# peter-seres/python-ray-tracer

Measured on AMD Instinct MI355X. Metric: Mrays/sec + frame time (ms) at 1920x1080, 8 spheres, depth=3, higher is better.
Workload: dtype f64

## Files before the change

python-ray-tracer_amd/csrc/mi355rt.hip:

```cpp
#include "../../include/mi355rt.h"
#include "rt_device.h"
#include "rt_bloom.h"
#include "rt_denoise.h"
#include "rt_denoise_var.h"
#include "rt_feedback.h"
#include "rt_film.h"
#include "rt_film_launch.h"
#include "rt_geometry.h"
#include "rt_guides.h"
#include "rt_launch.h"
#include "rt_plan.h"
#include "rt_scene.h"
#include "rt_streams.h"
#include "rt_temporal.h"

#include <cmath>
#include <cstdio>
#include <cstdlib>
#include <algorithm>
#include <array>
#include <cstring>
#include <memory>
#include <new>
#include <string>
// ... 40 lines not shown
        }
    };
    std::unique_ptr<Pipeline> pipe;
    int chunk_mode = -1;
    int cluster_min = rt::CLUSTER_MIN;
    int lanes_primary = 1;
    rt::PlanKnobs knobs;
    int render_chunks = 4;
    int log_kernels = 0;
    int remeasure = 24;
    struct Slot {
        hipStream_t stream = nullptr;
        Buf u8, f32;
    } slots[RT_RENDER_SLOTS];
    hipEvent_t ev0 = nullptr, ev1 = nullptr;
    Buf scene[RT_SCENE_RING];
    int scene_cur = 0;
    Buf pixel_loc, u8, f32;
    rt::SceneLayout lay;
    Buf texels[RT_SCENE_RING];
    bool have_scene = false;
    rt::View view;
    size_t lds_limit_set[rt::FAMILIES] = {};
    size_t guides_lds_set = 0;
    unsigned *tile_stats = nullptr;
    struct Feedback : rt::FeedbackSlot {
        Buf cost, gtmp, btmp, order[2];
    } fbs[RT_FEEDBACK_SLOTS];
    rt::FeedbackBook book;
    rt_ctx() { for (int i = 0; i < RT_FEEDBACK_SLOTS; ++i) book.slot[i] = &fbs[i]; }
    template <class F> void own_streams(F f)
    {
        if (stream) f(stream);
        for (Slot &sl : slots) if (sl.stream) f(sl.stream);
        if (pipe) pipe->streams(f);
    }
    ~rt_ctx()
    {
        for (auto &f : fbs)
            for (void *e : rt::release_events(f)) (void)hipEventDestroy((hipEvent_t)e);
        pipe.reset();
        own_streams([](hipStream_t s) { (void)hipStreamDestroy(s); });
        for (hipEvent_t e : {ev0, ev1}) if (e) (void)hipEventDestroy(e);
    }
    rt_stats stats = {};
    Buf counts;
// ... 37 lines not shown
int check_params(rt_ctx *ctx, const rt_params *p, int x0, int x1) { return refuse(ctx, rt::check_params(ctx->have_scene, ctx->view, ctx->lay, p, x0, x1)); }

hipStream_t stream_of(rt_ctx *ctx, void *stream) { return stream ? (hipStream_t)stream : ctx->stream; }

using StreamRecord = rt::StreamBook<Buf>::Record;

int stream_record(rt_ctx *ctx, hipStream_t stream, StreamRecord **out)
{
    const int rc = ctx->streams.record(stream, out);
    if (rc != RT_OK) return fail(ctx, rc, ctx->streams.NO_MEMORY);
    ctx->streams.reads_scene(**out, ctx->scene_cur);
    return RT_OK;
}

int raise_lds(rt_ctx *ctx, const void *const *fns, size_t n, size_t lds, size_t &set)
{
    if (lds <= 48 * 1024 || lds <= set) return RT_OK;
    for (size_t i = 0; i < n; ++i)
        if (fns[i]) RT_HIP(ctx, hipFuncSetAttribute(fns[i], hipFuncAttributeMaxDynamicSharedMemorySize, (int)lds));
    set = lds;
    return RT_OK;
}

using rt::Shape; using rt::SHAPES; using rt::NSHAPES; using rt::has_kernel;

template <rt::Family F, int I>
const void *kernel_at()
{
    constexpr Shape s = SHAPES[I];
    if constexpr (has_kernel(F, s))
        return (const void *)rt::render_kernel<s.aa, s.park, s.wpw, s.count, s.lat, s.mode, F>;
    else
        return nullptr;
}
template <rt::Family F, int... I>
std::array<const void *, NSHAPES> family_kernels(std::integer_sequence<int, I...>)
{
    return {kernel_at<F, I>()...};
}

constexpr std::make_integer_sequence<int, NSHAPES> ALL_SHAPES{};
const std::array<const void *, NSHAPES> KERNELS[rt::FAMILIES] = {
    family_kernels<rt::Family::PLAIN>(ALL_SHAPES), family_kernels<rt::Family::MAT>(ALL_SHAPES),
    family_kernels<rt::Family::REFR>(ALL_SHAPES),  family_kernels<rt::Family::SCAT>(ALL_SHAPES),
    family_kernels<rt::Family::SOFT>(ALL_SHAPES),  family_kernels<rt::Family::LENS>(ALL_SHAPES),
    family_kernels<rt::Family::LENS_SOFT>(ALL_SHAPES),
    family_kernels<rt::Family::TEX_SCAT>(ALL_SHAPES), family_kernels<rt::Family::TEX_SOFT>(ALL_SHAPES),
    family_kernels<rt::Family::TEX_LENS>(ALL_SHAPES), family_kernels<rt::Family::TEX_LENS_SOFT>(ALL_SHAPES),
    family_kernels<rt::Family::LIT_SCAT>(ALL_SHAPES), family_kernels<rt::Family::LIT_SOFT>(ALL_SHAPES),
    family_kernels<rt::Family::LIT_LENS>(ALL_SHAPES), family_kernels<rt::Family::LIT_LENS_SOFT>(ALL_SHAPES),
    family_kernels<rt::Family::SKY_SCAT>(ALL_SHAPES), family_kernels<rt::Family::SKY_SOFT>(ALL_SHAPES),
    family_kernels<rt::Family::SKY_LENS>(ALL_SHAPES), family_kernels<rt::Family::SKY_LENS_SOFT>(ALL_SHAPES),
};
static_assert(rt::FAMILIES == 19 && (int)rt::Family::TEX_LENS_SOFT == 10 && (int)rt::Family::LIT_LENS_SOFT == 14 &&
              (int)rt::Family::SKY_SCAT == 15 && (int)rt::Family::SKY_LENS_SOFT == 18,
              "KERNELS lists the families in enum order");

int stream_buffer(rt_ctx *ctx, Buf &b, hipStream_t stream, size_t bytes, bool sync)
{
    if (sync) RT_HIP(ctx, hipStreamSynchronize(stream));
    return ensure(ctx, b, bytes);
}

int acquire_tables(rt_ctx *ctx, StreamRecord &sr, const rt::KParams &k, const float **out)
{
    const hipStream_t stream = (hipStream_t)sr.stream;
    const rt::TableKey key = rt::table_key(ctx->scene_epoch, k.anchors, k.floor_anch, k.cam_o);
    const size_t bytes = rt::table_floats(k.S, k.NC, k.anchors, false, true, k.P) * sizeof(float);
    const rt::TableDecision d = ctx->streams.tables(sr, key, bytes);
    Buf &b = sr.buf[rt::BUF_TABLES0 + d.set];
    if (d.rebuild) {
        int rc = stream_buffer(ctx, b, stream, d.bytes, d.sync);
        if (rc != RT_OK) return rc;
        hipLaunchKernelGGL(rt::tables_kernel, dim3(1), dim3(rt::TABLE_THREADS), 0, stream, k, (float *)b.p);
        ctx->stats.table_builds++;
        RT_HIP(ctx, hipGetLastError());
// ... 111 lines not shown

int switch_order(rt_ctx *ctx, Feedback &f)
{
    if (!f.building) return RT_OK;
    const hipError_t q = hipEventQuery((hipEvent_t)f.done);
    if (q != hipSuccess) {
        (void)hipGetLastError();
        return RT_OK;
    }
    for (void *us : rt::switch_order(f)) {
        hipEvent_t ev = (hipEvent_t)rt::take_spare(f);
        if (!ev) RT_HIP(ctx, hipEventCreateWithFlags(&ev, hipEventDisableTiming));
        RT_HIP(ctx, hipEventRecord(ev, (hipStream_t)us));
        rt::add_fence(f, us, ev);
    }
    return RT_OK;
}

int launch_one(rt_ctx *ctx, rt::KParams &k, const rt::LaunchPlan &plan, const rt_geo_plan &g, const rt::OrderShape &os,
               Feedback *f, hipStream_t stream, int nframes, int64_t frame_stride)
{
    const Shape &sh = plan.shape;
    const int fi = (int)plan.family;
    const void *fn = KERNELS[fi][plan.index];
    const unsigned grid = (unsigned)g.blocks;
    if (ctx->log_kernels)
        std::fprintf(stderr, "mi355rt: render_kernel<%d, %d, %d, %d, %d, %d, (rt::Family)%d>\n", (int)sh.aa, (int)sh.park, sh.wpw, (int)sh.count,
                     (int)sh.lat, sh.mode, fi);
    int rc = raise_lds(ctx, KERNELS[fi].data(), KERNELS[fi].size(), plan.lds, ctx->lds_limit_set[fi]);
    if (rc != RT_OK) return rc;
    if (sh.count) {
        if (!ctx->counts.p) {
            rc = ensure(ctx, ctx->counts, RT_COUNT_WORDS * sizeof(unsigned long long));
            if (rc != RT_OK) return rc;
            RT_HIP(ctx, hipMemsetAsync(ctx->counts.p, 0, RT_COUNT_WORDS * sizeof(unsigned long long), stream));
        }
        k.ray_counts = (unsigned long long *)ctx->counts.p;
    }
    const rt::FeedbackLaunch d = f ? rt::decide_launch(*f, stream, ctx->epoch, ctx->remeasure) : rt::FeedbackLaunch{};
    if (d.read >= 0) k.order = (const unsigned *)f->order[d.read].p;
    if (d.measure) {
        const size_t words = (size_t)os.items * sizeof(unsigned);
        rc = ensure(ctx, f->cost, words);
        if (rc == RT_OK) rc = ensure(ctx, f->btmp, words);
        if (rc == RT_OK) rc = ensure(ctx, f->order[0], 2 * words);
        if (rc == RT_OK) rc = ensure(ctx, f->order[1], 2 * words);
        if (rc == RT_OK) rc = ensure(ctx, f->gtmp, words + sizeof(unsigned));
        if (rc != RT_OK) return rc;
        for (void *ev : d.wait) RT_HIP(ctx, hipStreamWaitEvent(stream, (hipEvent_t)ev, 0));
        k.cost = (unsigned *)f->cost.p;
    }
    rt::dispatch_part(k, nframes, grid, frame_stride, os);
// ... 45 lines not shown

int rt_create(rt_ctx **out, int device)
{
    if (!out) return fail(nullptr, RT_ERR_BAD_ARG, "ctx out-pointer is NULL");
    *out = nullptr;
    int n = 0;
    hipError_t e = hipGetDeviceCount(&n);
    if (e != hipSuccess || n <= 0)
        return fail(nullptr, RT_ERR_NO_DEVICE, std::string("no HIP device: ") + (e != hipSuccess ? hipGetErrorString(e) : "device count is 0"));
    if (device < 0 || device >= n) return fail(nullptr, RT_ERR_NO_DEVICE, "device index out of range");
    rt_ctx *ctx = new (std::nothrow) rt_ctx;
    if (!ctx) return fail(nullptr, RT_ERR_ALLOC, "out of host memory");
    ctx->device = device;
    if (const char *e = std::getenv("MI355RT_LANES_PRIMARY")) ctx->lanes_primary = std::atoi(e);
    if (const char *e = std::getenv("MI355RT_LANES_MINS")) ctx->knobs.lanes_min_spheres = std::atoi(e);
    if (const char *e = std::getenv("MI355RT_CLUSTER_MINS")) ctx->cluster_min = std::max(8, std::atoi(e));
    if (const char *e = std::getenv("MI355RT_CHUNK_MODE")) ctx->chunk_mode = std::atoi(e);
    if (const char *e = std::getenv("MI355RT_ORDER_GROUP")) { const int v = std::atoi(e); if (v >= 0 && v <= 6) ctx->knobs.order_group = v; }
    if (const char *e = std::getenv("MI355RT_REMEASURE")) ctx->remeasure = std::max(0, std::atoi(e));
    if (const char *e = std::getenv("MI355RT_F32_RECORDS")) ctx->knobs.f32_records = std::atoi(e) != 0;
    if (const char *e = std::getenv("MI355RT_WPW2_MAX_IMAGE")) ctx->knobs.wpw2_max_image = (size_t)std::max(0, std::atoi(e));
    if (const char *e = std::getenv("MI355RT_ORDER_TILES")) ctx->knobs.order_tiles = std::atoi(e) != 0;
    if (const char *e = std::getenv("MI355RT_LANES_PARK")) ctx->knobs.lanes_park = std::atoi(e) != 0;
    if (const char *e = std::getenv("MI355RT_LOG_KERNELS")) ctx->log_kernels = std::atoi(e) != 0;
    if (const char *e = std::getenv("MI355RT_SEQ_ORDER")) ctx->knobs.seq_order = std::atoi(e) != 0 ? 1 : 0;
    if (const char *e = std::getenv("MI355RT_CHUNKS")) { const int v = std::atoi(e); if (v >= 1 && v <= RT_RENDER_CHUNKS) ctx->render_chunks = v; }
    hipError_t s;
    if ((s = hipSetDevice(device)) != hipSuccess || (s = hipStreamCreateWithFlags(&ctx->stream, hipStreamNonBlocking)) != hipSuccess ||
        (s = hipEventCreate(&ctx->ev0)) != hipSuccess || (s = hipEventCreate(&ctx->ev1)) != hipSuccess) {
        std::string m = std::string("context setup: ") + hipGetErrorString(s);
        delete ctx;
        return fail(nullptr, RT_ERR_HIP, m);
    }
    {
        int cus = 0;
        if (hipDeviceGetAttribute(&cus, hipDeviceAttributeMultiprocessorCount, device) == hipSuccess && cus > 0) ctx->cu_count = cus;
        else (void)hipGetLastError();
    }
    *out = ctx;
    return RT_OK;
}

int rt_destroy(rt_ctx *ctx)
{
    if (!ctx) return RT_OK;
    (void)hipSetDevice(ctx->device);
// ... 742 lines not shown
    out->closest_queries = c[0]; out->shadow_traced = c[1]; out->shadow_skipped = c[2]; out->hits = c[3];
    for (int b = 0; b <= RT_MAX_DEPTH; ++b) { out->bounce_waves[b] = c[4 + 2 * b]; out->bounce_lanes[b] = c[5 + 2 * b]; }
    return RT_OK;
}

int rt_reset_stats(rt_ctx *ctx)
{
    if (!ctx) return RT_ERR_BAD_ARG;
    RT_HIP(ctx, hipSetDevice(ctx->device));
    if (ctx->counts.p) {
        RT_HIP(ctx, hipDeviceSynchronize());
        RT_HIP(ctx, hipMemset(ctx->counts.p, 0, RT_COUNT_WORDS * sizeof(unsigned long long)));
    }
    ctx->stats = rt_stats{};
    return RT_OK;
}

int rt_get_kernel_info(rt_ctx *ctx, rt_kernel_info *info)
{
    if (!ctx) return RT_ERR_BAD_ARG;
    if (!info) return fail(ctx, RT_ERR_BAD_ARG, "info is NULL");
    RT_HIP(ctx, hipSetDevice(ctx->device));
    hipFuncAttributes a;
    RT_HIP(ctx, hipFuncGetAttributes(&a, (const void *)rt::render_kernel<false, true, 2>));
    hipDeviceProp_t prop;
    RT_HIP(ctx, hipGetDeviceProperties(&prop, ctx->device));
    std::memset(info, 0, sizeof *info);
    info->vgprs = a.numRegs;
    info->lds_static = (int32_t)a.sharedSizeBytes;
    info->max_threads = a.maxThreadsPerBlock;
    info->wave_size = prop.warpSize;
    info->cu_count = prop.multiProcessorCount;
    info->clock_khz = prop.clockRate;
    return RT_OK;
}

}
```

python-ray-tracer_amd/csrc/rt_device.h:

```cpp
#pragma once
#include <hip/hip_runtime.h>
#include <stdint.h>
#include "rt_kparams.h"
#include "rt_math.h"
#include "rt_cull.h"
#include "rt_facing.h"
#include "rt_layout.h"

#pragma clang fp contract(off)

#ifndef RT_FAST_DIVSQRT
#define RT_FAST_DIVSQRT 1
#endif
#ifndef RT_FAST_NORMALIZE
#define RT_FAST_NORMALIZE 1
#endif
#ifndef RT_FACING_SKIP
#define RT_FACING_SKIP 1
#endif
#ifndef RT_DEFER_DIRECTION
#define RT_DEFER_DIRECTION 1
#endif
#ifndef RT_DEFER_SHADOW
#define RT_DEFER_SHADOW 1
// ... 298 lines not shown
            const bool self_culled = cand ? cull_origin(f4{cs[0], cs[1], cs[2], cs[3]}, q) : false;
            if (__builtin_amdgcn_ballot_w64(self_culled) != 0ull)
                return cull_mask_t<true, true>(lds, S, anchor, k0, n, q, self_culled ? self - k0 : -1);
        }
        return cull_mask_t<true, false>(lds, S, anchor, k0, n, q, -1);
    }
    add_origin(q, o, extent2);
    return cull_mask_t<false, false>(lds, S, anchor, k0, n, q, -1);
}

__device__ __forceinline__ unsigned long long cull_mask(const Lds &lds, int S, int anchor, int k0, int n,
                                                        const V3 &o, const V3 &R, float extent2, int self)
{
    return cull_mask(lds, S, anchor, k0, n, o, cull_dir32(R), extent2, self);
}


__device__ __forceinline__ int opaque(int x)
{
    asm volatile("" : "+s"(x));
    return x;
}

__device__ __forceinline__ int plane_code(const KParams &p, int k)
{
    unsigned c = p.plane_codes;
    asm volatile("" : "+s"(c));
    return k < 4 ? (int)(signed char)(c >> (8 * k)) : 0;
}

__device__ __forceinline__ void plane_den_num(const double *__restrict__ g, int code, const V3 &o, const V3 &d, double &den, double &num,
                                              bool no_negate = false)
{
    if (code == 0) {
        const V3 n{g[3], g[4], g[5]};
        den = dot3(d, n);
        const V3 LP{g[0] - o.x, g[1] - o.y, g[2] - o.z};
        num = dot3(LP, n);
    } else {
        const int a = code < 0 ? -code : code;
        double dc, lp;
        if (a == 1)      { dc = d.x; lp = g[0] - o.x; }
        else if (a == 2) { dc = d.y; lp = g[1] - o.y; }
        else             { dc = d.z; lp = g[2] - o.z; }
        if (code > 0 || no_negate) { den = dc; num = lp; } else { den = -dc; num = -lp; }
    }
}

struct SphHot { double x, y, z, r2; };
template <bool F32> __device__ __forceinline__ SphHot sphere_hot(const Lds &lds, int k)
{
// ... 301 lines not shown
    for (int k0 = 0; k0 < S; k0 += 64) {
      if (k0 > 0 && (live & ~occ) == 0ull) break;
      const int n = (S - k0 < 64) ? S - k0 : 64;
      unsigned long long mask = cull_mask(lds, S, canchor, k0, n, o, cull_dir32(IN_WINDOW ? d : Rg), p.extent2, self);
      mask &= (n == 64) ? ~0ull : ((1ull << n) - 1ull);
      RT_MARK(7);
      if (mask) {
        V3 R = Rg;
        if constexpr (IN_WINDOW) R = renormalize_unit_fast(d, pinned_here(e));
        const double a = dot3(R, R);
        const lanemask a_sane = lanes_where(a > 0.999999) & lanes_where(a < 1.000001);
        do {
          const int k = k0 + __builtin_ctzll(mask);
          mask &= mask - 1ull;
          occ |= sphere_any_mask<false>(lds, k, o, R, a, a_sane);
          if (mask && (live & ~occ) == 0ull) break;
        } while (mask);
      }
      RT_MARK(8);
    }
    return occ;
}

template <int MODE>
__device__ __forceinline__ void closest_hit(const Lds &lds, const KParams &p, const V3 &o, const V3 &d, int anchor,
                                            double &t_out, int &idx_out, int &type_out)
{
    const int P = opaque(p.P);
    const int S = p.S;
    constexpr bool F32 = MODE >= 1;
    double bestn = __builtin_inf();
    int bidx = -1;
    double aq;
    if (MODE < 2 && lds.defer) {
        const double e = unit_excess(d);
        const bool in_window = cull_reads_d(__builtin_amdgcn_ballot_w64(outside_unit_window(e)));
        RT_MARK(0);
        const int canchor = (opaque(p.anchors) > 0) ? anchor : -1;
        if (in_window) aq = closest_spheres<F32, true>(lds, p, S, canchor, o, d, e, bestn, bidx);
        else aq = closest_spheres<F32, false>(lds, p, S, canchor, o, d, e, bestn, bidx);
    } else {
    const V3 R = renormalize_unit(d);
    const double a = dot3(R, R);
    RT_MARK(0);
    const int canchor = (opaque(p.anchors) > 0) ? anchor : -1;
    if (MODE >= 2 && lds.NC > 0 && (canchor < 0 || p.lanes_primary)) {
        if (canchor >= 0) lanes_closest<true>(lds, p, canchor, o, R, a, bestn, bidx);
        else lanes_closest<false>(lds, p, -1, o, R, a, bestn, bidx);
    } else
    for (int k0 = 0; k0 < S; k0 += 64) {
      const int n = (S - k0 < 64) ? S - k0 : 64;
      unsigned long long mask = cull_mask(lds, S, canchor, k0, n, o, R, p.extent2, -1);
      mask &= (n == 64) ? ~0ull : ((1ull << n) - 1ull);
      RT_MARK(1);
      while (mask) {
        const int k = k0 + __builtin_ctzll(mask);
        mask &= mask - 1ull;
        sphere_closest<F32>(lds, p, k, o, R, a, bestn, bidx);
      }
      RT_MARK(2);
    }
    aq = a;
    }
    double best = 999.0;
    int idx = -1, type = HIT_NONE;
    if (bidx >= 0) {
        const double t = div_inrange(bestn, aq);
        if (best > t && t > 0.0) { best = t; idx = bidx; type = HIT_SPHERE; }
    }
    const double *pl = lds.recs() + (F32 ? 0 : opaque(p.S) * SPH_STRIDE);
    for (int k = 0; k < P; ++k) {
        const double *g = pl + k * PL_STRIDE;
        double den, num;
        plane_den_num(g, plane_code(p, k), o, d, den, num, lds.trim);
        if (!(__builtin_fabs(den) < 0.001)) {
            const double t = div_inrange(num, den);
            if (best > t && t > 0.0) { best = t; idx = k; type = HIT_PLANE; }
        }
    }
    t_out = best; idx_out = idx; type_out = type;
    RT_MARK(3);
}

__device__ __forceinline__ bool any_hit_masks(const Lds &lds, const KParams &p, const V3 &o, const V3 &d, int anchor, int self)
{
    const int P = opaque(p.P);
    const int S = p.S;
    const lanemask live = lanes_where(true);
    lanemask occ;
    if (RT_DEFER_SHADOW != 0 && lds.defer) {
        const double e = unit_excess(d);
        const bool in_window = cull_reads_d(__builtin_amdgcn_ballot_w64(outside_unit_window(e)));
        RT_MARK(6);
        const int canchor = (opaque(p.anchors) > 0) ? anchor : -1;
        if (in_window) occ = any_spheres_masks<true>(lds, p, S, canchor, o, d, e, self, live);
        else occ = any_spheres_masks<false>(lds, p, S, canchor, o, d, e, self, live);
    } else {
    const V3 R = renormalize_unit(d);
    const double a = dot3(R, R);
    RT_MARK(6);
    const int canchor = (opaque(p.anchors) > 0) ? anchor : -1;
    const lanemask a_sane = lanes_where(a > 0.999999) & lanes_where(a < 1.000001);
    occ = 0ull;
    for (int k0 = 0; k0 < S; k0 += 64) {
      if (k0 > 0 && (live & ~occ) == 0ull) break;
      const int n = (S - k0 < 64) ? S - k0 : 64;
      unsigned long long mask = cull_mask(lds, S, canchor, k0, n, o, R, p.extent2, self);
      mask &= (n == 64) ? ~0ull : ((1ull << n) - 1ull);
      RT_MARK(7);
      while (mask) {
        const int k = k0 + __builtin_ctzll(mask);
        mask &= mask - 1ull;
        occ |= sphere_any_mask<false>(lds, k, o, R, a, a_sane);
        if (mask && (live & ~occ) == 0ull) break;
      }
      RT_MARK(8);
    }
    }
    const double *pl = lds.recs() + opaque(p.S) * SPH_STRIDE;
    for (int k = 0; k < P; ++k) {
        if ((live & ~occ) == 0ull) break;
        const double *g = pl + k * PL_STRIDE;
        double den, num;
        plane_den_num(g, plane_code(p, k), o, d, den, num, true);
        const double an = __builtin_fabs(num), ad = __builtin_fabs(den);
        int sx = (int)(__builtin_bit_cast(unsigned long long, num) >> 32) ^ (int)(__builtin_bit_cast(unsigned long long, den) >> 32);
        asm("" : "+v"(sx));
        const lanemask ahead = lanes_where(!(ad < 0.001)) & lanes_where(sx >= 0) & lanes_where(an > 0.0);
        const lanemask sure = lanes_where(an < 998.0 * ad);
        occ |= ahead & sure;
        const lanemask edge = ahead & ~sure & ~occ;
        if (edge != 0ull) {
            bool h = false;
            if (lane_of(edge) && !(an > 1000.0 * ad)) { const double t = num / den; h = 999.0 > t && t > 0.0; }
            occ |= lanes_where(h);
        }
    }
    RT_MARK(9);
    return lane_of(occ);
}

template <int MODE>
__device__ __forceinline__ bool any_hit(const Lds &lds, const KParams &p, const V3 &o, const V3 &d, int anchor, int self, bool lanes = true)
{
    if (MODE == 0 && lds.trim) return any_hit_masks(lds, p, o, d, anchor, self);
    const int P = opaque(p.P);
    const int S = p.S;
    const V3 R = renormalize_unit(d);
    const double a = dot3(R, R);
    RT_MARK(6);
    const bool a_sane = (a > 0.999999 && a < 1.000001);
    bool occ = false;
    const int canchor = (opaque(p.anchors) > 0) ? anchor : -1;
    if (MODE >= 2 && lds.NC > 0 && lanes) {
        occ = (canchor >= 0) ? lanes_any<true>(lds, p, canchor, o, R, a, self) : lanes_any<false>(lds, p, -1, o, R, a, self);
    } else
    for (int k0 = 0; k0 < S; k0 += 64) {
      if (k0 > 0 && __builtin_amdgcn_ballot_w64(!occ) == 0ull) break;
      const int n = (S - k0 < 64) ? S - k0 : 64;
      unsigned long long mask = cull_mask(lds, S, canchor, k0, n, o, R, p.extent2, self);
      mask &= (n == 64) ? ~0ull : ((1ull << n) - 1ull);
      RT_MARK(7);
      while (mask) {
        const int k = k0 + __builtin_ctzll(mask);
        mask &= mask - 1ull;
        if (!occ) occ = sphere_any<(MODE >= 1)>(lds, k, o, R, a, a_sane);
        if (mask && __builtin_amdgcn_ballot_w64(!occ) == 0ull) break;
      }
      RT_MARK(8);
    }
    const double *pl = lds.recs() + (MODE >= 1 ? 0 : opaque(p.S) * SPH_STRIDE);
    for (int k = 0; k < P; ++k) {
        if (!occ) {
            const double *g = pl + k * PL_STRIDE;
            double den, num;
            plane_den_num(g, plane_code(p, k), o, d, den, num);
            if (!(__builtin_fabs(den) < 0.001)) {
                const double an = __builtin_fabs(num), ad = __builtin_fabs(den);
                const bool same_sign = (num > 0.0 && den > 0.0) || (num < 0.0 && den < 0.0);
                if (same_sign) {
                    if (an < 998.0 * ad) occ = true;
                    else if (!(an > 1000.0 * ad)) { const double t = num / den; if (999.0 > t && t > 0.0) occ = true; }
                }
            }
        }
    }
    RT_MARK(9);
    return occ;
}

template <bool COUNT> struct RayCount {
    __device__ __forceinline__ void closest(bool) {}
    __device__ __forceinline__ void hit(bool) {}
    __device__ __forceinline__ void shadow(bool, bool) {}
};
template <> struct RayCount<true> {
    unsigned n_closest = 0, n_issued = 0, n_skipped = 0, n_hit = 0;
    __device__ __forceinline__ void closest(bool alive) { n_closest += alive ? 1u : 0u; }
    __device__ __forceinline__ void hit(bool alive) { n_hit += alive ? 1u : 0u; }
// ... 138 lines not shown
        for (int i = 0; i < nhalo; ++i) q = q * q;
        g = V3{g.x + k[20] * q, g.y + k[21] * q, g.z + k[22] * q};
    }
    if (s >= k[16]) g = V3{g.x + k[17], g.y + k[18], g.z + k[19]};
    return g;
}

__device__ __forceinline__ int hit_slot(int type, int idx, int S) { return (type == HIT_SPHERE) ? idx : S + idx; }
template <bool NOREC> __device__ __forceinline__ int plane_base(int S) { return NOREC ? 0 : S * SPH_STRIDE; }
template <bool NOREC>
__device__ __forceinline__ void hit_normal(const Lds &lds, int type, int idx, int plb, const V3 &Pt, V3 &N, V3 &bN)
{
    if (type == HIT_SPHERE) {
        const SphHot g = sphere_hot<NOREC>(lds, idx);
        N = normalize3(V3{Pt.x - g.x, Pt.y - g.y, Pt.z - g.z});
        bN = V3{0.0002 * N.x, 0.0002 * N.y, 0.0002 * N.z};
    } else {
        const double *g = lds.recs() + plb + idx * PL_STRIDE;
        N = V3{g[6], g[7], g[8]};
        bN = V3{g[9], g[10], g[11]};
    }
}

template <bool PARK, int WGT, bool COUNT, int MODE, class MS>
__device__ __forceinline__ void trace_bounce(const Lds &lds, const KParams &p, bool &alive, int anchor,
                                             V3 &o, V3 &d, V3 &rgb, RayCount<COUNT> &cnt, MS &ms, int b = 0)
{
    constexpr bool NOREC = MODE >= 1;
    constexpr bool FACING_SKIP = RT_FACING_SKIP != 0 && MODE != 2;
    const int S = p.S, P = p.P, L = opaque(p.L);
    rgb = V3{0.0, 0.0, 0.0};
    double t = 999.0; int idx = -1, type = HIT_NONE;
    cnt.closest(alive);
    RT_MARK(11);
    if (alive) closest_hit<MODE>(lds, p, o, d, MS::lens ? -1 : anchor, t, idx, type);
    if constexpr (MS::sky) {
        if (alive && type == HIT_NONE) rgb = sky_color(p.scene + (size_t)p.lens.sky, d);
    }
    alive = alive && (type != HIT_NONE);
    cnt.hit(alive);
    if (alive) {
        V3 Pt{o.x + t * d.x, o.y + t * d.y, o.z + t * d.z};
        const int plb = plane_base<NOREC>(NOREC ? 0 : opaque(S));
        const int coff = (type == HIT_SPHERE) ? idx * SPH_STRIDE + 4 : plb + idx * PL_STRIDE + 12;
        volatile const lds_f64 *colp = (volatile const lds_f64 *)lds.recs() + coff;
        volatile const double *colf = (NOREC && type == HIT_SPHERE) ? p.scene + coff : lds.recs() + coff;
        typedef __attribute__((address_space(3))) float lds_f32;
        volatile const lds_f32 *col1 = nullptr;
        if constexpr (MODE == 1) col1 = (volatile const lds_f32 *)lds.col32 + 4 * ((type == HIT_SPHERE) ? idx : (int)padS(S, lds.NC) + idx);
        unsigned texi = 0u;
        if constexpr (MS::tex) texi = texel_of(p, hit_slot(type, idx, S), Pt);
        auto texel = [&](int c) -> double { return (double)((volatile const float *)p.lens.texels)[4 * (size_t)texi + c]; };
        V3 colr{0.0, 0.0, 0.0};
        if constexpr (!PARK && MS::tex) {
            const f4 tc = reinterpret_cast<const f4 *>(p.lens.texels)[texi];
            colr = V3{(double)tc[0], (double)tc[1], (double)tc[2]};
        }
        else if constexpr (!PARK) colr = (MODE == 1) ? V3{(double)col1[0], (double)col1[1], (double)col1[2]} : V3{colf[0], colf[1], colf[2]};
// ... 58 lines not shown
                const V3 dd = dpark.get();
                const V3 H = normalize3(V3{Ld.x - dd.x, Ld.y - dd.y, Ld.z - dd.z});
                const double s = dot3(N, H);
                if (s > 0.0) {
                    double q = s;
                    const int nsq = (int)lr[1];
#pragma unroll 1
                    for (int i = 0; i < nsq; ++i) q = q * q;
                    const double a = spec * q;
                    rgb = V3{rgb.x + a * er, rgb.y + a * eg, rgb.z + a * eb};
                }
              }
            }
        };
        for (int m = 0; m < L; ++m) {
            if constexpr (MS::soft) {
#pragma unroll 1
                for (int i = 0; i < ms.nsh; ++i) {
                    const V3 Ld = soft_Ld(m, i);
                    const double cN = dot3(Ld, N);
                    const double k = SLOT(LAMB) * cN;
                    RT_MARK(5);
                    if (k > 0.0 || (lit_row()[0] > 0.0 && cN > 0.0)) {
                        const bool occluded = any_hit<MODE>(lds, p, Pt, Ld, -1, self, true);
                        if (!occluded) lit_add(m, k, [&]() { return soft_Ld(again(m), i); });
                    }
                }
            } else {
                if constexpr (FACING_SKIP) {
                    const double *g = lt + m * LT_STRIDE;
                    const bool cert = rt_facing_certified_lamb(g[0] - Pt.x, g[1] - Pt.y, g[2] - Pt.z, N.x, N.y, N.z, p.facing_tau,
                                                               SLOT(LAMB));
                    if (__builtin_amdgcn_ballot_w64(!cert) == 0ull) { RT_MARK(5); continue; }
                }
                const V3 Ld = point_Ld(m);
                const double cN = dot3(Ld, N);
                const double k = SLOT(LAMB) * cN;
                RT_MARK(5);
                if (k > 0.0 || (lit_row()[0] > 0.0 && cN > 0.0)) {
                    const bool occluded = any_hit<MODE>(lds, p, Pt, Ld, 1 + m, self, anchor != 0 || p.lanes_primary);
                    if (!occluded) lit_add(m, k, [&]() { return point_Ld(again(m)); });
                }
            }
        }
        } else
        if constexpr (MS::soft) {
        for (int m = 0; m < L; ++m) {
            const double *g = lt + m * LT_STRIDE;
#pragma unroll 1
            for (int i = 0; i < ms.nsh; ++i) {
                const V3 Ld = soft_light_dir((unsigned)SLOT(LKEY), b, m, i, g, Pt);
                const double k = SLOT(LAMB) * dot3(Ld, N);
                RT_MARK(5);
                if (k > 0.0) {
                    const bool occluded = any_hit<MODE>(lds, p, Pt, Ld, -1, self, true);
                    if (!occluded) lambert_add(k, V3{1.0, 1.0, 1.0});
                }
            }
        }
        } else
        for (int m = 0; m < L; ++m) {
            const double *g = lt + m * LT_STRIDE;
            const V3 v{g[0] - Pt.x, g[1] - Pt.y, g[2] - Pt.z};
            double lamb;
            if constexpr (MS::mat) lamb = SLOT(LAMB); else lamb = p.lamb;
            if constexpr (FACING_SKIP) {
                bool cert;
                if constexpr (MS::mat) cert = rt_facing_certified_lamb(v.x, v.y, v.z, N.x, N.y, N.z, p.facing_tau, lamb);
                else cert = rt_facing_certified(v.x, v.y, v.z, N.x, N.y, N.z, p.facing_tau);
                if (__builtin_amdgcn_ballot_w64(!cert) == 0ull) {
                    cnt.shadow(true, false);
                    RT_MARK(5);
                    continue;
                }
            }
            const V3 Ld = normalize3(v);
            const double k = lamb * dot3(Ld, N);
            cnt.shadow(true, k > 0.0);
            RT_MARK(5);
            if (k > 0.0) {
                const bool occluded = any_hit<MODE>(lds, p, Pt, Ld, 1 + m, self, anchor != 0 || p.lanes_primary);
                if (!occluded) lambert_add(k, V3{1.0, 1.0, 1.0});
            }
        }
        d = dpark.get();
        if constexpr (MS::scat) {
            alive = refract_continue<WGT>(lds, ms, N, Pt, o, d, b < p.depth ? b : -1);
        } else if constexpr (MS::refr) {
            refract_continue<WGT>(lds, ms, N, Pt, o, d);
        } else {
        const V3 Rd = mirror_dir(d, N);
        o = V3{Pt.x + 0.0002 * Rd.x, Pt.y + 0.0002 * Rd.y, Pt.z + 0.0002 * Rd.z};
        d = Rd;
        }
        RT_MARK(10);
    }
}


template <bool PARK, int WGT, bool COUNT, int MODE, class MS>
__device__ __forceinline__ V3 sample(const Lds &lds, const KParams &p, bool alive, V3 o, V3 d, RayCount<COUNT> &cnt, MS &ms,
                                     unsigned key = 0u, unsigned lkey = 0u)
{
    Park3<PARK, WGT, MODE == 3> acc(lds.acc, 0, lds.wave);
    acc.set(V3{0.0, 0.0, 0.0});
    if constexpr (MS::mat) SLOT(W) = 1.0;
    if constexpr (MS::scat) SLOT(KEY) = (double)key;
    if constexpr (MS::soft) SLOT(LKEY) = (double)lkey;
    for (int b = 0; b <= p.depth; ++b) {
        if (__builtin_amdgcn_ballot_w64(alive) == 0ull) break;
        if constexpr (COUNT) {
            const unsigned long long am = __builtin_amdgcn_ballot_w64(alive);
            if ((threadIdx.x & 63u) == 0u && p.ray_counts) {
                atomicAdd(&p.ray_counts[4 + 2 * b], 1ull);
                atomicAdd(&p.ray_counts[5 + 2 * b], (unsigned long long)__builtin_popcountll(am));
            }
        }
        V3 rgb;
#ifdef RT_REGION_STATS
        ((volatile unsigned *)lds.reg)[(threadIdx.x >> 6) * 32 + 30] = b >= 2 ? 12u : 0u;
#endif
        trace_bounce<PARK, WGT, COUNT, MODE, MS>(lds, p, alive, b == 0 ? 0 : -1, o, d, rgb, cnt, ms, b);
        if (b == 0) acc.set(rgb);
        else {
            double wgt;
            if constexpr (MS::mat) wgt = SLOT(W); else wgt = p.refl_pow[b - 1];
            const V3 a = acc.get();
            acc.set(V3{a.x + wgt * rgb.x, a.y + wgt * rgb.y, a.z + wgt * rgb.z});
        }
        if constexpr (MS::mat) {
            if (alive) {
                volatile lds_f64 *w = &SLOT(W);
                *w = *w * SLOT(REFL);
            }
        }
    }
    return acc.get();
}

__device__ __forceinline__ V3 pixel_P(const KParams &p, int x, int y)
{
    if (p.pixel_loc) {
        const size_t wh = (size_t)p.w * p.h, o = (size_t)x * p.h + y;
        return V3{p.pixel_loc[o], p.pixel_loc[wh + o], p.pixel_loc[2 * wh + o]};
    }
// ... 158 lines not shown
        const double az = a ? lt[(a - 1) * LT_STRIDE + 2] : p.cam_o[2];
        const double lx = ax - c[0], ly = ay - c[1], lz = az - c[2];
        const double ll = lx * lx + ly * ly + lz * lz;
        t[0] = (float)lx; t[1] = (float)ly; t[2] = (float)lz;
        t[3] = anchored_tau(ll, c[3], p.floor_anch);
    }
}

template <Family F, int WSLOT, bool FRESH>
__device__ __forceinline__ MatState<F, WSLOT, FRESH> mat_state(double *matl, int M, int nsh = 1)
{
    typedef __attribute__((address_space(3))) double lds_d;
    typedef MatState<F, WSLOT, FRESH> MS;
    if constexpr (MS::mat) return MS{(unsigned)(size_t)(lds_d *)(matl + 1), (unsigned)(size_t)(lds_d *)(matl + 1 + MS::COLS * M), nsh};
    else return {};
}

__device__ __forceinline__ void tile_xy(const KParams &p, int tile, int &tx, int &ty)
{
    tx = div_by(tile, p.tiles_y, p.tiles_y_magic, p.tiles_y_shift);
    ty = tile - tx * p.tiles_y;
}

template <bool AA, bool PARK, int WPW, bool COUNT = false, bool LAT = false, int MODE = 0, Family F = Family::PLAIN>
__global__ __launch_bounds__(64 * WPW, MODE >= 2 ? RT_W_LANES : (AA ? (PARK ? RT_W_AAPARK : 4) : (PARK ? RT_W_PARK : 5))) void render_kernel(const KParams p)
{
    constexpr int WG_THREADS = 64 * WPW, WAVES_PER_WG = WPW;
    constexpr bool M2 = MODE >= 2;
    constexpr bool NOREC = MODE >= 1;
    constexpr bool MAT = has_mat(F), SCAT = has_scat(F), SOFT = has_soft(F), LENS = has_lens(F), TEX = has_tex(F);
    const int nrec = (int)lds_doubles(NOREC ? 0 : p.S, p.P, p.L);
    const double *rec_src = p.scene + (NOREC ? (size_t)p.S * SPH_STRIDE : 0);
    double *accum = lds_raw + nrec;
    int *offw = reinterpret_cast<int *>(accum + lds_slots(AA, PARK, M2, F) * WG_THREADS);
    float *sph32 = reinterpret_cast<float *>(offw + lds_offset_words(PARK, WG_THREADS));
    const TableLayout tl = table_layout(p.S, p.NC, p.anchors, p.P);
    const bool LANES = MODE >= 2 && p.anchors > 0;
    float *tab = sph32 + tl.tab;
    float *csph32 = LANES ? nullptr : sph32 + tl.csph32;
    float *ctab = sph32 + tl.ctab;
    float *cbox = sph32 + tl.cbox;
    const size_t ntab = MODE == 1 ? tl.total_col : (LANES ? tl.total_lanes : tl.total);
    unsigned *wgstat = reinterpret_cast<unsigned *>(sph32 + ntab);
    if (threadIdx.x == 0) { wgstat[0] = 0u; wgstat[1] = 0u; }
    {
        for (int i = threadIdx.x; i < nrec; i += WG_THREADS) lds_raw[i] = rec_src[i];
        const int nf4 = (int)(ntab / 4);
// ... 44 lines not shown
    const int y = ty * TILE + (lane & 7);
    bool inb = (x < p.x1) && (y < p.h);
    if constexpr (LAT) inb = inb && ((((x | y) & 1) == 0) || (x >= 1 && x <= p.w - 2 && y >= 1 && y <= p.h - 2));
    const int xc = inb ? x : p.x0, yc = inb ? y : 0;
    typedef __attribute__((address_space(3))) int lds_i32;
    constexpr bool OFF_REMAT = PARK && MODE == 3;
    volatile lds_i32 *offp = OFF_REMAT ? nullptr : (volatile lds_i32 *)offw + threadIdx.x;
    if constexpr (PARK && !OFF_REMAT) *offp = inb ? (x - p.x0) * p.h + y : -1;

    const V3 o{p.cam_o[0], p.cam_o[1], p.cam_o[2]};
    RayCount<COUNT> cnt;
    constexpr int WSLOT = lds_slots(AA, PARK, M2, Family::PLAIN);
    auto ms = mat_state<F, WSLOT, !PARK || MODE == 3>(matl, nmat, nsh);
    const unsigned sseed = SCAT ? p.seed : 0u;
    double R, G, B;
    if constexpr (!AA) {
        unsigned key = 0u, lkey = 0u;
        if constexpr (SCAT) key = LAT ? scatter_key((unsigned)xc, (unsigned)yc, 0u, sseed) : scatter_key(2u * xc, 2u * yc, 0u, sseed);
        if constexpr (SOFT) lkey = LAT ? soft_key((unsigned)xc, (unsigned)yc, 0u, sseed) : soft_key(2u * xc, 2u * yc, 0u, sseed);
        const V3 P0 = LAT ? lattice_P(p, xc, yc) : pixel_P(p, xc, yc);
        V3 ro = o, rd;
        if constexpr (LENS) lens_ray(p, LAT ? (unsigned)xc : 2u * xc, LAT ? (unsigned)yc : 2u * yc, 0u, P0, ro, rd);
        else rd = primary_dir(p, P0);
        const V3 c = sample<PARK, WG_THREADS, COUNT, MODE, decltype(ms)>(lds, p, inb, ro, rd, cnt, ms, key, lkey);
        R = c.x; G = c.y; B = c.z;
    } else {
        const bool stoch = (p.aa == 2);
        const bool interior = !stoch && inb && x >= 1 && x <= p.w - 2 && y >= 1 && y <= p.h - 2;
        const int ntaps = stoch ? p.spp : ((__builtin_amdgcn_ballot_w64(interior) != 0ull) ? 9 : 1);
        constexpr unsigned NBX = 0x8858u, NBY = 0x0A25u;
        Park3<PARK && !M2, WG_THREADS> taps(lds.acc, 2);
#pragma unroll 1
        for (int tap = 0; tap < ntaps; ++tap) {
            const V3 Pp = pixel_P(p, xc, yc);
            V3 Pt = Pp;
            unsigned key = 0u, lkey = 0u;
            unsigned lx = 2u * xc, ly = 2u * yc;
            if constexpr (SCAT) key = scatter_key(2u * xc, 2u * yc, stoch ? (unsigned)tap : 0u, sseed);
            if constexpr (SOFT) lkey = soft_key(2u * xc, 2u * yc, stoch ? (unsigned)tap : 0u, sseed);
            if (stoch) {
                const unsigned hh = jitter_hash((unsigned)xc, (unsigned)yc, (unsigned)tap, p.seed);
                const double u = (double)(hh & 0xFFFFu) * 0x1p-16 + (0x1p-17 - 0.5);
                const double v = (double)(hh >> 16) * 0x1p-16 + (0x1p-17 - 0.5);
                Pt = V3{Pp.x, Pp.y + u * p.dy, Pp.z + v * p.dz};
            } else if (tap) {
                const int k = tap - 1;
                const int ddx = (int)((NBX >> (2 * k)) & 3u) - 1, ddy = (int)((NBY >> (2 * k)) & 3u) - 1;
                const V3 Pn = pixel_P(p, interior ? x + ddx : xc, interior ? y + ddy : yc);
                Pt = V3{0.5 * Pp.x + 0.5 * Pn.x, 0.5 * Pp.y + 0.5 * Pn.y, 0.5 * Pp.z + 0.5 * Pn.z};
                if constexpr (SCAT) key = scatter_key((unsigned)(2 * xc + ddx), (unsigned)(2 * yc + ddy), 0u, sseed);
                if constexpr (SOFT) lkey = soft_key((unsigned)(2 * xc + ddx), (unsigned)(2 * yc + ddy), 0u, sseed);
                if constexpr (LENS) { lx = (unsigned)(2 * xc + ddx); ly = (unsigned)(2 * yc + ddy); }
            }
            V3 ro = o, rd;
            if constexpr (LENS) lens_ray(p, lx, ly, stoch ? (unsigned)tap : 0u, Pt, ro, rd);
            else rd = primary_dir(p, Pt);
            const V3 s = sample<PARK, WG_THREADS, COUNT, MODE, decltype(ms)>(lds, p, (tap && !stoch) ? interior : inb, ro, rd, cnt, ms, key, lkey);
            if (tap == 0) taps.set(s);
            else if (stoch) { const V3 a = taps.get(); taps.set(V3{a.x + s.x, a.y + s.y, a.z + s.z}); }
            else if (interior) { const V3 a = taps.get(); taps.set(V3{a.x + s.x, a.y + s.z, a.z + s.y}); }
        }
        { const V3 a = taps.get(); R = a.x; G = a.y; B = a.z; }
        if (stoch) { const double n = (double)p.spp; R = R / n; G = G / n; B = B / n; }
        else if (interior) { R = R / 9; G = G / 9; B = B / 9; }
    }

    long long off;
    if constexpr (OFF_REMAT) {
        const int l2 = (int)fresh_lane();
        const int x2 = p.x0 + tx * TILE + (l2 >> 3), y2 = ty * TILE + (l2 & 7);
        bool inb2 = (x2 < p.x1) && (y2 < p.h);
        if constexpr (LAT) inb2 = inb2 && ((((x2 | y2) & 1) == 0) || (x2 >= 1 && x2 <= p.w - 2 && y2 >= 1 && y2 <= p.h - 2));
        off = inb2 ? (long long)((x2 - p.x0) * p.h + y2) : -1ll;
    } else if constexpr (PARK) off = *offp; else off = inb ? (long long)(x - p.x0) * p.h + y : -1ll;
    if (off >= 0) {
        if constexpr (LAT) {
            double *q = p.out_f64 + off * 3;
            q[0] = R; q[1] = G; q[2] = B;
        } else {
            const long long fo = opaque(p.nframes) > 1 ? (long long)div_by((int)blockIdx.x, p.bpf, p.bpf_magic, p.bpf_shift) * p.frame_stride : 0ll;
// ... 156 lines not shown
```

python-ray-tracer_amd/csrc/rt_plan.h:

```cpp
#pragma once
#include "rt_layout.h"
#include "rt_scene.h"
#include "rt_geometry.h"

#include <algorithm>
#include <cstddef>

namespace rt {

struct PlanKnobs {
    int lanes_min_spheres = 161;
    int f32_records = 1;
    size_t wpw2_max_image = 4608;
    int lanes_park = 1;
    int order_group = -1;
    int order_tiles = 1;
    int seq_order = -1;
};

inline Family family_of(const SceneLayout &s, double lens_a)
{
    using F = Family;
    const bool lens = lens_a > 0.0, soft = s.soft_n > 0;
    if (s.M <= 0) return F::PLAIN;
    if (s.sky)
        return lens ? (soft ? F::SKY_LENS_SOFT : F::SKY_LENS) : (soft ? F::SKY_SOFT : F::SKY_SCAT);
    if (s.lit)
        return lens ? (soft ? F::LIT_LENS_SOFT : F::LIT_LENS) : (soft ? F::LIT_SOFT : F::LIT_SCAT);
    if (s.T > 0)
        return lens ? (soft ? F::TEX_LENS_SOFT : F::TEX_LENS) : (soft ? F::TEX_SOFT : F::TEX_SCAT);
    if (lens) return soft ? F::LENS_SOFT : F::LENS;
    return block_family(s.M, s.mat_cols, soft);
}

struct Shape {
    bool aa, park;
    int wpw;
    bool count, lat;
    int mode;
    constexpr bool operator==(const Shape &o) const
    {
        return aa == o.aa && park == o.park && wpw == o.wpw && count == o.count && lat == o.lat && mode == o.mode;
    }
};

constexpr Shape SHAPES[] = {
    {false, false, 2, false, false, 0}, {false, true, 2, false, false, 0}, {true, false, 2, false, false, 0}, {true, true, 2, false, false, 0},
    {false, false, 4, false, false, 0}, {false, true, 4, false, false, 0}, {true, false, 4, false, false, 0}, {true, true, 4, false, false, 0},
    {false, false, 4, false, false, 1}, {false, true, 4, false, false, 1},
    {false, false, 2, false, true, 0}, {false, true, 2, false, true, 0}, {false, false, 4, false, true, 0}, {false, true, 4, false, true, 0},
    {false, false, 4, false, true, 1}, {false, true, 4, false, true, 1},
    {false, false, 4, false, false, 2}, {false, true, 4, false, false, 2}, {true, false, 4, false, false, 2}, {true, true, 4, false, false, 3},
    {false, false, 4, false, true, 2}, {false, true, 4, false, true, 2},
    {false, false, 4, true, false, 0}, {true, false, 4, true, false, 0}, {false, false, 4, true, true, 0},
};
constexpr int NSHAPES = sizeof SHAPES / sizeof SHAPES[0];

constexpr bool has_kernel(Family f, const Shape &s)
{
    return (!s.count || f == Family::PLAIN) && !(has_refr(f) && s.park && s.mode < 2);
}

constexpr int PARK_WAVES = 24;
constexpr size_t CU_LDS = 160 * 1024;

constexpr bool missing_kernels_never_park()
{
    for (int fi = 0; fi < FAMILIES; ++fi)
        for (const Shape &s : SHAPES) {
            const Family f = (Family)fi;
            if (s.count || has_kernel(f, s)) continue;
            const size_t wgt = 64 * s.wpw;
            const size_t least = lds_slots(s.aa, true, s.mode >= 2, f) * wgt * sizeof(double) +
                                 wgt * sizeof(int) + 16;
            if (!s.park || s.mode >= 2 || least * (PARK_WAVES / s.wpw) <= CU_LDS) return false;
        }
    return true;
}
static_assert(missing_kernels_never_park(), "the parking rule can pick a render kernel that is not compiled");

inline int anchors_of(const SceneLayout &lay)
{
    const size_t table = (size_t)(lay.L + 1) * (padS(lay.S, lay.NC) + pad4(lay.NC)) * CULL_STRIDE * sizeof(float);
// ... 86 lines not shown
```

Measured before the change: 216,000.

## Add ground-plane specialized render kernels with compile-time plane count and code

Adds a GROUND template variant of the render kernel and its intersection helpers. It is selected when the scene has exactly one plane with code 3 in the PLAIN family. Inside it the plane count and plane code become compile-time constants, so the plane loop and code decode can be unrolled and simplified. This means more kernel instantiations, which costs compile time and binary size, and it adds a host-side dispatch path with an env knob to turn it off.

```diff
diff --git a/python-ray-tracer_amd/csrc/mi355rt.hip b/python-ray-tracer_amd/csrc/mi355rt.hip
--- a/python-ray-tracer_amd/csrc/mi355rt.hip
+++ b/python-ray-tracer_amd/csrc/mi355rt.hip
@@ -86,6 +86,7 @@
     bool have_scene = false;
     rt::View view;
     size_t lds_limit_set[rt::FAMILIES] = {};
+    size_t ground_lds_set = 0;
     size_t guides_lds_set = 0;
     unsigned *tile_stats = nullptr;
     struct Feedback : rt::FeedbackSlot {
@@ -169,14 +170,14 @@
     return RT_OK;
 }
 
-using rt::Shape; using rt::SHAPES; using rt::NSHAPES; using rt::has_kernel;
-
-template <rt::Family F, int I>
+using rt::Shape; using rt::SHAPES; using rt::NSHAPES; using rt::has_kernel; using rt::has_ground_kernel;
+
+template <rt::Family F, int I, bool GROUND = false>
 const void *kernel_at()
 {
     constexpr Shape s = SHAPES[I];
-    if constexpr (has_kernel(F, s))
-        return (const void *)rt::render_kernel<s.aa, s.park, s.wpw, s.count, s.lat, s.mode, F>;
+    if constexpr (GROUND ? has_ground_kernel(F, s) : has_kernel(F, s))
+        return (const void *)rt::render_kernel<s.aa, s.park, s.wpw, s.count, s.lat, s.mode, F, GROUND>;
     else
         return nullptr;
 }
@@ -184,6 +185,11 @@
 std::array<const void *, NSHAPES> family_kernels(std::integer_sequence<int, I...>)
 {
     return {kernel_at<F, I>()...};
+}
+template <int... I>
+std::array<const void *, NSHAPES> ground_kernels(std::integer_sequence<int, I...>)
+{
+    return {kernel_at<rt::Family::PLAIN, I, true>()...};
 }
 
 constexpr std::make_integer_sequence<int, NSHAPES> ALL_SHAPES{};
@@ -199,6 +205,8 @@
     family_kernels<rt::Family::SKY_SCAT>(ALL_SHAPES), family_kernels<rt::Family::SKY_SOFT>(ALL_SHAPES),
     family_kernels<rt::Family::SKY_LENS>(ALL_SHAPES), family_kernels<rt::Family::SKY_LENS_SOFT>(ALL_SHAPES),
 };
+const std::array<const void *, NSHAPES> GROUND_KERNELS = ground_kernels(ALL_SHAPES);
+const std::array<const void *, NSHAPES> &kernels_of(int fi, bool ground) { return ground ? GROUND_KERNELS : KERNELS[fi]; }
 static_assert(rt::FAMILIES == 19 && (int)rt::Family::TEX_LENS_SOFT == 10 && (int)rt::Family::LIT_LENS_SOFT == 14 &&
               (int)rt::Family::SKY_SCAT == 15 && (int)rt::Family::SKY_LENS_SOFT == 18,
               "KERNELS lists the families in enum order");
@@ -356,12 +364,15 @@
 {
     const Shape &sh = plan.shape;
     const int fi = (int)plan.family;
-    const void *fn = KERNELS[fi][plan.index];
+    const bool ground = rt::ground_plane(ctx->lay, ctx->knobs, plan.family, sh.count ? RT_FLAG_COUNT_RAYS : 0) && has_ground_kernel(plan.family, sh);
+    const std::array<const void *, NSHAPES> &kernels = kernels_of(fi, ground);
+    const void *fn = kernels[plan.index];
+    if (!fn) return fail(ctx, RT_ERR_STATE, "no render kernel for this launch");
     const unsigned grid = (unsigned)g.blocks;
     if (ctx->log_kernels)
-        std::fprintf(stderr, "mi355rt: render_kernel<%d, %d, %d, %d, %d, %d, (rt::Family)%d>\n", (int)sh.aa, (int)sh.park, sh.wpw, (int)sh.count,
-                     (int)sh.lat, sh.mode, fi);
-    int rc = raise_lds(ctx, KERNELS[fi].data(), KERNELS[fi].size(), plan.lds, ctx->lds_limit_set[fi]);
+        std::fprintf(stderr, "mi355rt: render_kernel<%d, %d, %d, %d, %d, %d, (rt::Family)%d>%s\n", (int)sh.aa, (int)sh.park, sh.wpw, (int)sh.count,
+                     (int)sh.lat, sh.mode, fi, ground ? " ground" : "");
+    int rc = raise_lds(ctx, kernels.data(), kernels.size(), plan.lds, ground ? ctx->ground_lds_set : ctx->lds_limit_set[fi]);
     if (rc != RT_OK) return rc;
     if (sh.count) {
         if (!ctx->counts.p) {
@@ -453,6 +464,7 @@
     if (const char *e = std::getenv("MI355RT_WPW2_MAX_IMAGE")) ctx->knobs.wpw2_max_image = (size_t)std::max(0, std::atoi(e));
     if (const char *e = std::getenv("MI355RT_ORDER_TILES")) ctx->knobs.order_tiles = std::atoi(e) != 0;
     if (const char *e = std::getenv("MI355RT_LANES_PARK")) ctx->knobs.lanes_park = std::atoi(e) != 0;
+    if (const char *e = std::getenv("MI355RT_GROUND_PLANE")) ctx->knobs.ground_plane = std::atoi(e) != 0;
     if (const char *e = std::getenv("MI355RT_LOG_KERNELS")) ctx->log_kernels = std::atoi(e) != 0;
     if (const char *e = std::getenv("MI355RT_SEQ_ORDER")) ctx->knobs.seq_order = std::atoi(e) != 0 ? 1 : 0;
     if (const char *e = std::getenv("MI355RT_CHUNKS")) { const int v = std::atoi(e); if (v >= 1 && v <= RT_RENDER_CHUNKS) ctx->render_chunks = v; }
@@ -1241,7 +1253,10 @@
     if (!info) return fail(ctx, RT_ERR_BAD_ARG, "info is NULL");
     RT_HIP(ctx, hipSetDevice(ctx->device));
     hipFuncAttributes a;
-    RT_HIP(ctx, hipFuncGetAttributes(&a, (const void *)rt::render_kernel<false, true, 2>));
+    const bool ground = ctx->have_scene && rt::ground_plane(ctx->lay, ctx->knobs, rt::Family::PLAIN, 0);
+    const void *fn = ground ? (const void *)rt::render_kernel<false, true, 2, false, false, 0, rt::Family::PLAIN, true>
+                            : (const void *)rt::render_kernel<false, true, 2>;
+    RT_HIP(ctx, hipFuncGetAttributes(&a, fn));
     hipDeviceProp_t prop;
     RT_HIP(ctx, hipGetDeviceProperties(&prop, ctx->device));
     std::memset(info, 0, sizeof *info);
diff --git a/python-ray-tracer_amd/csrc/rt_device.h b/python-ray-tracer_amd/csrc/rt_device.h
--- a/python-ray-tracer_amd/csrc/rt_device.h
+++ b/python-ray-tracer_amd/csrc/rt_device.h
@@ -344,11 +344,18 @@
     return x;
 }
 
-__device__ __forceinline__ int plane_code(const KParams &p, int k)
-{
+template <bool GROUND = false> __device__ __forceinline__ int plane_code(const KParams &p, int k)
+{
+    if constexpr (GROUND) return 3;
     unsigned c = p.plane_codes;
     asm volatile("" : "+s"(c));
     return k < 4 ? (int)(signed char)(c >> (8 * k)) : 0;
+}
+
+template <bool GROUND = false> __device__ __forceinline__ int plane_count(const KParams &p)
+{
+    if constexpr (GROUND) return 1;
+    else return opaque(p.P);
 }
 
 __device__ __forceinline__ void plane_den_num(const double *__restrict__ g, int code, const V3 &o, const V3 &d, double &den, double &num,
@@ -696,11 +703,11 @@
     return occ;
 }
 
-template <int MODE>
+template <int MODE, bool GROUND = false>
 __device__ __forceinline__ void closest_hit(const Lds &lds, const KParams &p, const V3 &o, const V3 &d, int anchor,
                                             double &t_out, int &idx_out, int &type_out)
 {
-    const int P = opaque(p.P);
+    const int P = plane_count<GROUND>(p);
     const int S = p.S;
     constexpr bool F32 = MODE >= 1;
     double bestn = __builtin_inf();
@@ -746,7 +753,7 @@
     for (int k = 0; k < P; ++k) {
         const double *g = pl + k * PL_STRIDE;
         double den, num;
-        plane_den_num(g, plane_code(p, k), o, d, den, num, lds.trim);
+        plane_den_num(g, plane_code<GROUND>(p, k), o, d, den, num, lds.trim);
         if (!(__builtin_fabs(den) < 0.001)) {
             const double t = div_inrange(num, den);
             if (best > t && t > 0.0) { best = t; idx = k; type = HIT_PLANE; }
@@ -756,9 +763,10 @@
     RT_MARK(3);
 }
 
+template <bool GROUND = false>
 __device__ __forceinline__ bool any_hit_masks(const Lds &lds, const KParams &p, const V3 &o, const V3 &d, int anchor, int self)
 {
-    const int P = opaque(p.P);
+    const int P = plane_count<GROUND>(p);
     const int S = p.S;
     const lanemask live = lanes_where(true);
     lanemask occ;
@@ -796,7 +804,7 @@
         if ((live & ~occ) == 0ull) break;
         const double *g = pl + k * PL_STRIDE;
         double den, num;
-        plane_den_num(g, plane_code(p, k), o, d, den, num, true);
+        plane_den_num(g, plane_code<GROUND>(p, k), o, d, den, num, true);
         const double an = __builtin_fabs(num), ad = __builtin_fabs(den);
         int sx = (int)(__builtin_bit_cast(unsigned long long, num) >> 32) ^ (int)(__builtin_bit_cast(unsigned long long, den) >> 32);
         asm("" : "+v"(sx));
@@ -814,11 +822,11 @@
     return lane_of(occ);
 }
 
-template <int MODE>
+template <int MODE, bool GROUND = false>
 __device__ __forceinline__ bool any_hit(const Lds &lds, const KParams &p, const V3 &o, const V3 &d, int anchor, int self, bool lanes = true)
 {
-    if (MODE == 0 && lds.trim) return any_hit_masks(lds, p, o, d, anchor, self);
-    const int P = opaque(p.P);
+    if (MODE == 0 && lds.trim) return any_hit_masks<GROUND>(lds, p, o, d, anchor, self);
+    const int P = plane_count<GROUND>(p);
     const int S = p.S;
     const V3 R = renormalize_unit(d);
     const double a = dot3(R, R);
@@ -848,7 +856,7 @@
         if (!occ) {
             const double *g = pl + k * PL_STRIDE;
             double den, num;
-            plane_den_num(g, plane_code(p, k), o, d, den, num);
+            plane_den_num(g, plane_code<GROUND>(p, k), o, d, den, num);
             if (!(__builtin_fabs(den) < 0.001)) {
                 const double an = __builtin_fabs(num), ad = __builtin_fabs(den);
                 const bool same_sign = (num > 0.0 && den > 0.0) || (num < 0.0 && den < 0.0);
@@ -1033,7 +1041,7 @@
     }
 }
 
-template <bool PARK, int WGT, bool COUNT, int MODE, class MS>
+template <bool PARK, int WGT, bool COUNT, int MODE, class MS, bool GROUND = false>
 __device__ __forceinline__ void trace_bounce(const Lds &lds, const KParams &p, bool &alive, int anchor,
                                              V3 &o, V3 &d, V3 &rgb, RayCount<COUNT> &cnt, MS &ms, int b = 0)
 {
@@ -1044,7 +1052,7 @@
     double t = 999.0; int idx = -1, type = HIT_NONE;
     cnt.closest(alive);
     RT_MARK(11);
-    if (alive) closest_hit<MODE>(lds, p, o, d, MS::lens ? -1 : anchor, t, idx, type);
+    if (alive) closest_hit<MODE, GROUND>(lds, p, o, d, MS::lens ? -1 : anchor, t, idx, type);
     if constexpr (MS::sky) {
         if (alive && type == HIT_NONE) rgb = sky_color(p.scene + (size_t)p.lens.sky, d);
     }
@@ -1149,7 +1157,7 @@
                     const double k = SLOT(LAMB) * cN;
                     RT_MARK(5);
                     if (k > 0.0 || (lit_row()[0] > 0.0 && cN > 0.0)) {
-                        const bool occluded = any_hit<MODE>(lds, p, Pt, Ld, -1, self, true);
+                        const bool occluded = any_hit<MODE, GROUND>(lds, p, Pt, Ld, -1, self, true);
                         if (!occluded) lit_add(m, k, [&]() { return soft_Ld(again(m), i); });
                     }
                 }
@@ -1165,7 +1173,7 @@
                 const double k = SLOT(LAMB) * cN;
                 RT_MARK(5);
                 if (k > 0.0 || (lit_row()[0] > 0.0 && cN > 0.0)) {
-                    const bool occluded = any_hit<MODE>(lds, p, Pt, Ld, 1 + m, self, anchor != 0 || p.lanes_primary);
+                    const bool occluded = any_hit<MODE, GROUND>(lds, p, Pt, Ld, 1 + m, self, anchor != 0 || p.lanes_primary);
                     if (!occluded) lit_add(m, k, [&]() { return point_Ld(again(m)); });
                 }
             }
@@ -1180,7 +1188,7 @@
                 const double k = SLOT(LAMB) * dot3(Ld, N);
                 RT_MARK(5);
                 if (k > 0.0) {
-                    const bool occluded = any_hit<MODE>(lds, p, Pt, Ld, -1, self, true);
+                    const bool occluded = any_hit<MODE, GROUND>(lds, p, Pt, Ld, -1, self, true);
                     if (!occluded) lambert_add(k, V3{1.0, 1.0, 1.0});
                 }
             }
@@ -1206,7 +1214,7 @@
             cnt.shadow(true, k > 0.0);
             RT_MARK(5);
             if (k > 0.0) {
-                const bool occluded = any_hit<MODE>(lds, p, Pt, Ld, 1 + m, self, anchor != 0 || p.lanes_primary);
+                const bool occluded = any_hit<MODE, GROUND>(lds, p, Pt, Ld, 1 + m, self, anchor != 0 || p.lanes_primary);
                 if (!occluded) lambert_add(k, V3{1.0, 1.0, 1.0});
             }
         }
@@ -1225,7 +1233,7 @@
 }
 
 
-template <bool PARK, int WGT, bool COUNT, int MODE, class MS>
+template <bool PARK, int WGT, bool COUNT, int MODE, class MS, bool GROUND = false>
 __device__ __forceinline__ V3 sample(const Lds &lds, const KParams &p, bool alive, V3 o, V3 d, RayCount<COUNT> &cnt, MS &ms,
                                      unsigned key = 0u, unsigned lkey = 0u)
 {
@@ -1247,7 +1255,7 @@
 #ifdef RT_REGION_STATS
         ((volatile unsigned *)lds.reg)[(threadIdx.x >> 6) * 32 + 30] = b >= 2 ? 12u : 0u;
 #endif
-        trace_bounce<PARK, WGT, COUNT, MODE, MS>(lds, p, alive, b == 0 ? 0 : -1, o, d, rgb, cnt, ms, b);
+        trace_bounce<PARK, WGT, COUNT, MODE, MS, GROUND>(lds, p, alive, b == 0 ? 0 : -1, o, d, rgb, cnt, ms, b);
         if (b == 0) acc.set(rgb);
         else {
             double wgt;
@@ -1452,7 +1460,7 @@
     ty = tile - tx * p.tiles_y;
 }
 
-template <bool AA, bool PARK, int WPW, bool COUNT = false, bool LAT = false, int MODE = 0, Family F = Family::PLAIN>
+template <bool AA, bool PARK, int WPW, bool COUNT = false, bool LAT = false, int MODE = 0, Family F = Family::PLAIN, bool GROUND = false>
 __global__ __launch_bounds__(64 * WPW, MODE >= 2 ? RT_W_LANES : (AA ? (PARK ? RT_W_AAPARK : 4) : (PARK ? RT_W_PARK : 5))) void render_kernel(const KParams p)
 {
     constexpr int WG_THREADS = 64 * WPW, WAVES_PER_WG = WPW;
@@ -1543,7 +1551,7 @@
         V3 ro = o, rd;
         if constexpr (LENS) lens_ray(p, LAT ? (unsigned)xc : 2u * xc, LAT ? (unsigned)yc : 2u * yc, 0u, P0, ro, rd);
         else rd = primary_dir(p, P0);
-        const V3 c = sample<PARK, WG_THREADS, COUNT, MODE, decltype(ms)>(lds, p, inb, ro, rd, cnt, ms, key, lkey);
+        const V3 c = sample<PARK, WG_THREADS, COUNT, MODE, decltype(ms), GROUND>(lds, p, inb, ro, rd, cnt, ms, key, lkey);
         R = c.x; G = c.y; B = c.z;
     } else {
         const bool stoch = (p.aa == 2);
@@ -1576,7 +1584,7 @@
             V3 ro = o, rd;
             if constexpr (LENS) lens_ray(p, lx, ly, stoch ? (unsigned)tap : 0u, Pt, ro, rd);
             else rd = primary_dir(p, Pt);
-            const V3 s = sample<PARK, WG_THREADS, COUNT, MODE, decltype(ms)>(lds, p, (tap && !stoch) ? interior : inb, ro, rd, cnt, ms, key, lkey);
+            const V3 s = sample<PARK, WG_THREADS, COUNT, MODE, decltype(ms), GROUND>(lds, p, (tap && !stoch) ? interior : inb, ro, rd, cnt, ms, key, lkey);
             if (tap == 0) taps.set(s);
             else if (stoch) { const V3 a = taps.get(); taps.set(V3{a.x + s.x, a.y + s.y, a.z + s.z}); }
             else if (interior) { const V3 a = taps.get(); taps.set(V3{a.x + s.x, a.y + s.z, a.z + s.y}); }
diff --git a/python-ray-tracer_amd/csrc/rt_plan.h b/python-ray-tracer_amd/csrc/rt_plan.h
--- a/python-ray-tracer_amd/csrc/rt_plan.h
+++ b/python-ray-tracer_amd/csrc/rt_plan.h
@@ -16,6 +16,7 @@
     int order_group = -1;
     int order_tiles = 1;
     int seq_order = -1;
+    int ground_plane = 1;
 };
 
 inline Family family_of(const SceneLayout &s, double lens_a)
@@ -59,6 +60,25 @@
 constexpr bool has_kernel(Family f, const Shape &s)
 {
     return (!s.count || f == Family::PLAIN) && !(has_refr(f) && s.park && s.mode < 2);
+}
+
+constexpr Shape NO_GROUND_TWIN[] = {
+    {false, false, 2, false, false, 0}, {true, false, 2, false, false, 0},
+    {false, false, 4, false, false, 1}, {false, false, 4, false, true, 1},
+    {false, false, 4, false, false, 2}, {false, false, 4, false, true, 2},
+};
+constexpr bool has_ground_kernel(Family f, const Shape &s)
+{
+    if (f != Family::PLAIN || s.count) return false;
+    for (const Shape &n : NO_GROUND_TWIN)
+        if (n == s) return false;
+    return true;
+}
+
+inline bool ground_plane(const SceneLayout &lay, const PlanKnobs &kn, Family fam, int flags)
+{
+    const int code0 = (int)(signed char)(lay.plane_codes & 0xffu);
+    return kn.ground_plane != 0 && fam == Family::PLAIN && !(flags & RT_FLAG_COUNT_RAYS) && lay.P == 1 && code0 == 3;
 }
 
 constexpr int PARK_WAVES = 24;
```

Result: faster. 223,400, median of 6 (+3.5%).
